# uci-cbcl/RP-Net

Hardware: AMD Instinct MI355X
Metric: support/query pairs/sec (fwd+bwd, 1-shot 256x256, T=5) (higher is better)
Workload: dtype f32

## Files before the change

rpnet_amd/csrc/bn.hip:

```cpp
#include <stdlib.h>

#include "common.h"
#include "lds_dma.h"
#include "split_bf16.h"

namespace rpnet {

struct BnGeom {
    int C4;
    int rows_it;
    int nblk;
    int rows_blk;
};

struct YSrc {
    const float* y;
};
__device__ __forceinline__ f32x4 load_y4(const YSrc s, const size_t off, const int) {
    return *reinterpret_cast<const f32x4*>(s.y + off);
}

static int bn_max_blocks(int C) { const int m = 131072 / C; return m < 256 ? 256 : (m > 1024 ? 1024 : m); }

static BnGeom bn_geom(long R, int C) {
// ... 176 lines not shown
                                                            const int C, const float sqrt_n, float* __restrict__ s_out) {
    RPNET_PASS_PRIORITY();
    __shared__ float red4[4];
    float m = 0.f;
    for (int c = threadIdx.x; c < C; c += 256) m = fmaxf(m, fabsf(gamma[c]) * sqrt_n + fabsf(beta[c]));
    m = block_max256(m, red4);
    if (threadIdx.x == 0) *s_out = pow2_scale(m);
}

template <int NP>
__global__ __launch_bounds__(256) void bn_relu_split_kernel(const YSrc ysrc, const float* __restrict__ scale,
                                                             const float* __restrict__ shift, float* __restrict__ z,
                                                             unsigned short* __restrict__ zs, size_t total8, int C8,
                                                             size_t group8, size_t plane_elems, const float* __restrict__ gamma,
                                                             const float* __restrict__ beta, const float sqrt_n,
                                                             float* __restrict__ s_out, const FastDiv fc, const FastDiv fg) {
    RPNET_PASS_PRIORITY();
    float inv_s = 1.f;
    if (NP <= 2) {
        __shared__ float red4[4];
        float m = 0.f;
        for (int c = threadIdx.x; c < C8 * 8; c += 256) m = fmaxf(m, fabsf(gamma[c]) * sqrt_n + fabsf(beta[c]));
        const float sc = pow2_scale(block_max256(m, red4));
        if (blockIdx.x == 0 && threadIdx.x == 0) *s_out = sc;
        inv_s = 1.f / sc;
    }
    for (size_t i = (size_t)blockIdx.x * 256 + threadIdx.x; i < total8; i += (size_t)gridDim.x * 256) {
        const int c8 = (int)fc.mod((unsigned)i);
        const int g = (int)fg.div((unsigned)i);
        const float* sc = scale + (size_t)(g * C8 + c8) * 8;
        const float* sh = shift + (size_t)(g * C8 + c8) * 8;
        float v[8];
#pragma unroll
        for (int hh = 0; hh < 2; ++hh) {
// ... 246 lines not shown
            for (int k = 0; k < 4; ++k) {
                const float m = fmaxf(fmaxf(a[k] * s4[k] + h4[k], b[k] * s4[k] + h4[k]), fmaxf(c[k] * s4[k] + h4[k], d[k] * s4[k] + h4[k]));
                o[k] = fmaxf(m, 0.f);
                v[hh * 4 + k] = o[k];
            }
            if (zp) reinterpret_cast<f32x4*>(zp)[i * 2 + hh] = o;
        }
        if (NP <= 2) {
#pragma unroll
            for (int k = 0; k < 8; ++k) v[k] *= inv_s;
        }
        u32x4 pl[NP];
        split8<NP>(v, pl);
#pragma unroll
        for (int p = 0; p < NP; ++p) *reinterpret_cast<u32x4*>(zs + p * plane_elems + i * 8) = pl[p];
    }
}

__device__ __forceinline__ int pool_argmax(const float a0, const float a1, const float a2, const float a3, float& best) {
    int q = 0; best = a0;
    if (a1 > best) { best = a1; q = 1; }
    if (a2 > best) { best = a2; q = 2; }
    if (a3 > best) { best = a3; q = 3; }
    return q;
}

template <int WIN>
__global__ __launch_bounds__(256) void bn_bwd_partial_pool(const float* __restrict__ dp, const YSrc ysrc,
                                                            const float* __restrict__ scale, const float* __restrict__ shift,
                                                            const float* __restrict__ mean, const float* __restrict__ invstd,
// ... 281 lines not shown
        else if (planes == 2) RPNET_BN_POOL(2);
        else RPNET_BN_POOL(1);
#undef RPNET_BN_POOL
        return check_launch("bn_relu_pool");
    }
    const size_t total4 = (size_t)N * HW * C / 4, group4 = total4 / groups;
    RPNET_REQUIRE(total4 < kIndex32, RPNET_ERR_SHAPE, "bn: %zu 16-byte elements do not fit the 32-bit index arithmetic of the passes", total4);
    if (z_split) {
        RPNET_REQUIRE(planes >= 1 && planes <= 3 && C % 8 == 0, RPNET_ERR_SHAPE, "bn_relu: split planes=%d C=%d", planes, C);
        const size_t total8 = total4 / 2, pe = (size_t)N * HW * C;
        RPNET_REQUIRE(planes == 3 || (gamma && beta && split_scale), RPNET_ERR_ARG,
                      "bn_relu: fp16 planes (1 or 2) need gamma, beta and the scale output");
        const float sqrt_n = sqrtf((float)((size_t)(N / groups) * HW)) * 1.0001f;
        if (planes == 3)
            hipLaunchKernelGGL(bn_relu_split_kernel<3>, dim3(elt_grid(total8)), dim3(256), 0, (hipStream_t)stream, ysrc, scale,
                               shift, z, (unsigned short*)z_split, total8, C / 8, group4 / 2, pe, gamma, beta, sqrt_n, split_scale, FastDiv(C / 8), FastDiv((unsigned)(group4 / 2)));
        else if (planes == 2)
            hipLaunchKernelGGL(bn_relu_split_kernel<2>, dim3(elt_grid(total8)), dim3(256), 0, (hipStream_t)stream, ysrc, scale,
                               shift, z, (unsigned short*)z_split, total8, C / 8, group4 / 2, pe, gamma, beta, sqrt_n, split_scale, FastDiv(C / 8), FastDiv((unsigned)(group4 / 2)));
        else
            hipLaunchKernelGGL(bn_relu_split_kernel<1>, dim3(elt_grid(total8)), dim3(256), 0, (hipStream_t)stream, ysrc, scale,
                               shift, z, (unsigned short*)z_split, total8, C / 8, group4 / 2, pe, gamma, beta, sqrt_n, split_scale, FastDiv(C / 8), FastDiv((unsigned)(group4 / 2)));
        return check_launch("bn_relu_split");
    }
    RPNET_REQUIRE(!split_scale || (gamma && beta), RPNET_ERR_ARG, "bn_relu: the tensor scale needs gamma and beta");
    hipLaunchKernelGGL(bn_relu_kernel, dim3(elt_grid(total4)), dim3(256), 0, (hipStream_t)stream, ysrc, scale, shift, z,
                       total4, C / 4, group4, gamma, beta, sqrtf((float)((size_t)(N / groups) * HW)) * 1.0001f, split_scale, FastDiv(C / 4),
                       FastDiv((unsigned)group4));
    return check_launch("bn_relu");
}

extern "C" int rpnet_bn_act_scale(const float* gamma, const float* beta, float* split_scale, int N, int HW, int C, int groups,
                                  rpnet_stream_t stream) {
    using namespace rpnet;
    RPNET_REQUIRE(gamma && beta && split_scale && groups >= 1 && C > 0, RPNET_ERR_ARG, "bn_act_scale: bad argument");
    hipLaunchKernelGGL(bn_act_scale_kernel, dim3(1), dim3(256), 0, (hipStream_t)stream, gamma, beta, C,
                       sqrtf((float)((size_t)(N / groups) * HW)) * 1.0001f, split_scale);
    return check_launch("bn_act_scale");
}

extern "C" int rpnet_bn_bwd(const float* dz, const float* y, const float* gamma, const float* scale, const float* shift,
                            const float* mean, const float* invstd, float* dy, void* dy_split, int planes, float* split_scale,
                            float* dgamma, float* dbeta, int N, int HW, int C, int groups, int accumulate,
                            const double* given_partial, const float* given_pmax, int given_rows, int pool_w, void* workspace,
                            size_t workspace_bytes, const float* y_dec, int y_dec_stride, rpnet_stream_t stream) {
    using namespace rpnet;
    (void)gamma;
    RPNET_REQUIRE(!y_dec && !y_dec_stride, RPNET_ERR_ARG, "bn_bwd: y_dec / y_dec_stride are reserved (must be NULL / 0)");
    const YSrc ysrc{y};
    RPNET_REQUIRE(dz && scale && shift && mean && invstd && dgamma && dbeta && workspace, RPNET_ERR_ARG, "bn_bwd: null pointer");
    RPNET_REQUIRE(y || (given_partial && !dy && !dy_split), RPNET_ERR_ARG, "bn_bwd: y is NULL but a pass that reads it was asked for");
    RPNET_REQUIRE(!dy_split || (planes >= 1 && planes <= 3 && C % 8 == 0), RPNET_ERR_SHAPE, "bn_bwd: split planes=%d C=%d",
                  planes, C);
// ... 140 lines not shown
```

rpnet_amd/functional.py:

```python
import collections
import contextlib
import ctypes as C
import os

import torch
from torch.autograd import Function
from torch.autograd.function import once_differentiable

from . import hip
from .hip import ConvDesc, call, ptr, query

BN_EPS = 1e-5
BN_MOMENTUM = 0.1

_ASYNC = {"on": False, "side": {}, "pending": set(), "queued": False, "fifo": [], "keep": []}

_MODES = {"f32": (0, False, 0), "bf16x3": (3, False, 0), "f16x2": (3, True, 2), "f16": (3, True, 1)}
_CORR_PRED_PLANES = True
_MATH = {}


def set_conv_math(mode):
    _MATH["mode"] = mode
    _MATH["planes"], _MATH["f16"], _MATH["f16_planes"] = _MODES[mode]
# ... 320 lines not shown
        if device is None or dv == device:
            for k in out:
                out[k] += pd[k]
    return out


def _empty(shape, like, dtype=torch.float32):
    return torch.empty(shape, device=like.device, dtype=dtype)


def _ws(nbytes, like):
    return torch.empty((max(int(nbytes), 16) + 7) // 8, device=like.device, dtype=torch.float64)


class Operand:
    __slots__ = ("x", "p16", "pbf", "scale", "planes_only", "deferred", "masked")

    def __init__(self, x, p16=None, pbf=None, scale=None, planes_only=False, deferred=None, masked=None):
        self.x, self.p16, self.pbf, self.scale = x, p16, pbf, scale
        self.deferred = deferred
        self.masked = masked
        self.planes_only = planes_only

    def values(self):
        if self.planes_only:
            raise RuntimeError("rpnet_amd: this operand exists as fp16 planes only (its producer was told that its single "
                               "consumer is a 3x3 convolution on fp16 planes); a consumer asked for the fp32 values")
        return self.x

    @property
    def shape(self):
        return self.x.shape

    def derive(self, x):
        return Operand(x, scale=self.scale)


_WGRAD_DEFER = 1
_EVAL_SPLITK = True
_POOL_FUSE = True
_CONV1_BN_FUSE = True
_CONV1_RECOMP = True
_UP4 = True
_MASK_SKIP = os.environ.get("RPNET_MASK_SKIP", "1") == "1"


_SKIP_STATS = None


def _set_skip(d, mask, mode, halo, N, H, W, on=None):
    if (_MASK_SKIP if on is None else on) and mask is not None and mode in (1, 2):
        if _SKIP_STATS is not None:
            d._skip_ws = torch.full((max(N * H * W // 128, 16),), 255, device=mask.device, dtype=torch.uint8)
            _SKIP_STATS.append(d._skip_ws)
        else:
            d._skip_ws = torch.empty(max(N * H * W // 128, 16), device=mask.device, dtype=torch.uint8)
        d.skip_mask, d.skip_mode, d.skip_halo, d.skip_ws = ptr(mask), mode, halo, ptr(d._skip_ws)
        ARITH[("zero_tile_skip", "armed")] += 1

# ... 50 lines not shown
        return None
    masked = in_scale is not None and in_mode
    fp = _MATH["f16_planes"]

    def ready(op):
        return op.p16 is not None and op.p16.shape[1:] == op.x.shape and op.p16.shape[0] == fp

    if op1 is None and not masked and ready(op0):
        return op0.p16, None, s0, None
    pre = op0.masked
    if (op1 is None and masked and pre is not None and pre[0] is in_scale and pre[1] == in_mode and pre[2].shape[0] == fp
            and pre[2].dtype == torch.float16):
        return pre[2], None, s0, None
    if two_scales and op1 is not None and not masked and ready(op0) and ready(op1):
        return op0.p16, op1.p16, s0, s1
    xs0, s = split_f16(op0.values(), s0, s1, in_scale if masked else None, in_mode if masked else 0)
    xs1 = split_f16(op1.values(), s0, s1, want_scale=False)[0] if op1 is not None else None
    if op1 is None and not masked:
        op0.p16 = xs0
    return xs0, xs1, s, None


class PackedWeight:

    def __init__(self, weight, split=None, pool=None):
        cout, cin, kh, kw = weight.shape
        self._pool = pool
        self.taps = kh * kw
        if split is None:
            self.off0, self.split, self.off1, self.cin_pad = 0, cin, cin, cin
# ... 201 lines not shown

def _dgrad_desc(pw, dys, sdy, dy, g0, g1, N, H, W, out_scale=None, out_mode=0, up4=False, skippable=False, skip_on=None):
    if dys is None:
        return _desc(dy, None, pw.wd, None, None, 0, g0, g1, N, H, W, pw.taps, 0, out_scale=out_scale, out_mode=out_mode)
    np_ = dys.shape[0]
    pk = pw.up4_packs(np_) if up4 else pw.split_packs(np_)
    dd = _desc(dys, None, pk[1], None, None, 0, g0, g1, N, H, W, pw.taps, 1 if up4 else 0, out_scale=out_scale, out_mode=out_mode)
    dd.split_planes = np_
    if np_ <= 2:
        dd.acc_scale_col, dd.acc_scale_x = ptr(pk[3]), ptr(sdy)
        if skippable:
            _set_skip(dd, out_scale, out_mode, 0, N, H, W, skip_on)
    return dd


_Req = collections.namedtuple("_Req", "z_unused pool pool_req defer_act eval_grad")


class _Produced:
    __slots__ = ("p16", "pbf", "scale", "planes_only", "deferred", "pooled")

    def __init__(self):
        self.p16 = self.pbf = self.scale = self.deferred = None
        self.planes_only = self.pooled = False


_State = collections.namedtuple("_State", "shape groups bias beta bn_eval pool pw upsample in_mode xs sx sx1 up4 async_on skip_on")


def _save_state(ctx, saved=None, shape=None, groups=1, bias=None, beta=None, bn_eval=False, pool=False, pw=None, upsample=0, in_mode=0, plan=None):
    if saved is None:
        ctx.st = None
        return
    ctx.save_for_backward(*saved)
    split = plan is not None and plan.planes
    ctx.st = _State(shape, groups, bias, beta, bn_eval, pool, pw, upsample, in_mode, plan.xs if split else None,
                    plan.sx if split else None, plan.sx1 if split else None, plan is not None and plan.kind == "up4", _ASYNC["on"], _MASK_SKIP)

# ... 46 lines not shown
             BN_EPS, ptr(stats[0]), ptr(stats[1]), ptr(stats[2]), ptr(stats[3]), ptr(ws), wsb)
    _order_done(gamma.data_ptr())
    return stats


def _bn_output(y, stats, shape, groups, gamma, beta, out_split, req, res, pool_ok, conv1=None):
    N, H, W, cout = shape
    planes_out = out_split in (True, "corr")
    want16 = _want16(cout, out_split)
    np_out = 0
    if planes_out and cout % 32 == 0 and _MATH["planes"]:
        np_out = _MATH["f16_planes"] if want16 else _MATH["planes"]
    pool = res.pooled = bool(pool_ok and np_out > 0 and out_split is True and H % 2 == 0 and W % 2 == 0)
    Hz, Wz = (H // 2, W // 2) if pool else (H, W)
    dev = gamma.device
    zs = torch.empty((np_out, N, Hz, Wz, cout), device=dev, dtype=torch.float16 if np_out <= 2 else torch.bfloat16) if np_out else None
    sz = torch.empty(1, device=dev, dtype=torch.float32) if want16 else None
    if req.z_unused and want16 and np_out and (pool or not req.pool_req):
        z = torch.empty(1, device=dev, dtype=torch.float32).expand(N, Hz, Wz, cout)
        res.planes_only = True
    else:
        z = torch.empty((N, Hz, Wz, cout), device=dev, dtype=torch.float32)
    if req.defer_act and not (pool or np_out or want16 or res.planes_only) and conv1 is None and groups == 1:
        res.deferred = (y, stats[0], stats[1])
    elif conv1 is not None:
        if not (res.planes_only and np_out):
            raise RuntimeError("rpnet_amd: the first layer was run without its pre-BatchNorm tensor but its output is not planes-only")
        call("rpnet_conv1_bn_relu", ptr(conv1[0]), ptr(conv1[1]), ptr(conv1[2]), ptr(stats[0]), ptr(stats[1]), None, ptr(zs), np_out,
             ptr(gamma), ptr(beta), ptr(sz), N, H, W, cout, groups)
        ARITH[("bn_relu", "first layer made again from the image")] += 1
# ... 319 lines not shown
        if fuse:
            call("rpnet_conv1_wgrad_bn", ptr(x0), ptr(dz), ptr(y), ptr(stats), coef, ptr(dw), N, H, W, cout, groups, ptr(ws2), wb, *again)
        else:
            call("rpnet_conv1_wgrad", ptr(x0), ptr(dy), ptr(dw), N, H, W, cout, ptr(ws2), wb)
        dw = _accumulate_direct(weight, dw, st.async_on)
        dx0 = None
        if ctx.needs_input_grad[0]:
            dx0 = _empty(x0.shape, dz)
            call("rpnet_conv1_dgrad_bn", ptr(dz), ptr(y), ptr(stats), coef, ptr(weight), again[1], ptr(x0) if y is None else None,
                 ptr(dx0), N, H, W, cout, groups)
        db = _bias_grad(bias, gamma, stats, dbeta, st.bn_eval, st.async_on)
        return dx0, dw, db, dgamma, dbeta, None, None, None, None


def conv_bn_relu_op(x0, conv, bn, cache, training, x1=None, in_scale=None, in_mode=0, groups=1, upsample=False, split=None,
                    out_split=True, z_unused=False, pool=False, defer_act=False):
    op0, op1 = as_operand(x0), as_operand(x1)
    w = conv.weight
    x1t = None if op1 is None else op1.x
    eval_grad = not training and torch.is_grad_enabled() and any(
        t is not None and t.requires_grad for t in (op0.x, x1t, in_scale, w, conv.bias, bn.weight, bn.bias))
    req = _Req(bool(z_unused) and training and w.shape[0] % 64 == 0, bool(pool) and training and _POOL_FUSE, bool(pool),
               bool(defer_act) and training and not out_split, eval_grad)
    res = _Produced()
    bnbuf = (bn.running_mean, bn.running_var, bn.num_batches_tracked if training else None)
    if w.shape[1] == 1 and w.shape[2] == 3:
        if x1t is not None or in_scale is not None or upsample:
            raise RuntimeError("rpnet_amd: the first-layer convolution takes one plain source (no second source, mask or up-sampling)")
        z = Conv1BnRelu.apply(op0.x, w, conv.bias, bn.weight, bn.bias, bnbuf, (training, groups, out_split), req, res)
    else:
        pw = cache.get(w, split)
        z = ConvBnRelu.apply(op0.x, x1t, in_scale, w, conv.bias, bn.weight, bn.bias, bnbuf, pw,
                             (training, groups, 1 if upsample else 0, in_mode, out_split), (op0, op1), req, res)
    out = Operand(z, res.p16, res.pbf, res.scale, res.planes_only, res.deferred)
    if pool and not res.pooled:
        out = maxpool2(out)
    return out


def conv_bn_relu(x0, conv, bn, cache, training, **kw):
    return conv_bn_relu_op(x0, conv, bn, cache, training, **kw).x


class ConvRelu(Function):

    @staticmethod
    def forward(ctx, x, weight, bias, pw, relu, dilation):
        hip.require_gpu(x, weight)
        N, H, W, _ = x.shape
# ... 122 lines not shown
                dst.zero_()
                continue
            for i in range(0, len(live), 15):
                chunk = ([dst] if i else []) + live[i:i + 15]
                if len(chunk) == 1:
                    dst.copy_(chunk[0])
                else:
                    arr = (C.c_void_p * len(chunk))(*[t.data_ptr() for t in chunk])
                    call("rpnet_sum_n", arr, len(chunk), ptr(dst), dst.numel())
        return out, None, None, None


class PoolSkip(Function):

    @staticmethod
    def forward(ctx, z):
        N, H, W, Cc = z.shape
        out = _empty((N, H // 2, W // 2, Cc), z)
        call("rpnet_maxpool2_fwd", ptr(z), ptr(out), N, H, W, Cc)
        ctx.save_for_backward(z)
        return z.view_as(z), out

    @staticmethod
    @once_differentiable
    def backward(ctx, dskip, dpool):
        if dpool is None:
            return dskip
        (z,) = ctx.saved_tensors
        N, H, W, Cc = z.shape
        dz = torch.empty_like(z)
        call("rpnet_maxpool2_bwd", ptr(z), ptr(dpool.contiguous()), None if dskip is None else ptr(dskip.contiguous()), ptr(dz),
             N, H, W, Cc)
        return dz


def pool_skip(op):
    op = as_operand(op)
    z, pooled = PoolSkip.apply(op.values())
    return Operand(z, p16=op.p16, pbf=op.pbf, scale=op.scale), op.derive(pooled)


class MaxPool2(Function):

    @staticmethod
    def forward(ctx, z):
        N, H, W, Cc = z.shape
        out = _empty((N, H // 2, W // 2, Cc), z)
        call("rpnet_maxpool2_fwd", ptr(z), ptr(out), N, H, W, Cc)
        ctx.save_for_backward(z)
        return out

    @staticmethod
    @once_differentiable
# ... 389 lines not shown
```

rpnet_amd/hip.py:

```python
import ctypes as C
import os

import torch

_LIB_PATH = os.environ.get("RPNET_LIB_PATH") or os.path.join(os.path.dirname(os.path.abspath(__file__)), "librpnet_hip.so")
_lib = None

vp, ci, cf, cs, cd = C.c_void_p, C.c_int, C.c_float, C.c_size_t, C.c_double


class ConvDesc(C.Structure):
    _fields_ = [("x0", vp), ("x1", vp), ("C0", ci), ("C1", ci), ("w", vp), ("bias", vp), ("in_scale", vp),
                ("in_scale_mode", ci), ("y0", vp), ("y1", vp), ("Co0", ci), ("Co1", ci), ("ep_scale", vp),
                ("ep_shift", vp), ("ep_relu", ci), ("out_scale", vp), ("out_scale_mode", ci), ("accumulate", ci),
                ("N", ci), ("H", ci), ("W", ci), ("taps", ci), ("upsample", ci), ("groups", ci), ("dilation", ci), ("stats_partial", vp), ("split_planes", ci), ("y_split", vp), ("split_out_planes", ci),
                ("acc_scale_col", vp), ("acc_scale_x", vp), ("acc_scale_dy", vp), ("bnb_y", vp), ("bnb_stats", vp), ("bnb_partial", vp), ("bnb_pmax", vp), ("bnb_groups", ci),
                ("acc_scale_x1", vp), ("out_absmax", vp), ("tune", ci), ("y_split_scale", vp), ("splitk_ws", vp), ("splitk_ws_bytes", cs),
                ("skip_mask", vp), ("skip_mode", ci), ("skip_halo", ci), ("skip_ws", vp), ("tile_skip", vp),
                ("y_enc", vp), ("y_enc_stride", ci)]


PACK_MAX = 24


# ... 134 lines not shown
    "rpnet_surface_workspace_bytes": (cs, [ci, ci, ci]),
    "rpnet_surface_tally": (ci, [vp, ci, vp, ci, ci, ci, ci, ci, vp, C.c_int64, vp, C.c_int64, C.c_int64, vp, cs, vp]),
}
SURFACE_ABI_SYMBOLS = tuple(_SURFACE_SIGS)
SURFACE_ABI_VERSION = 1

_CC_SIGS = {
    "rpnet_cc_abi_version": (ci, []),
    "rpnet_cc_workspace_bytes": (cs, [ci, ci, ci]),
    "rpnet_cc_label": (ci, [vp, ci, ci, ci, ci, ci, ci, vp, vp, C.c_int64, C.c_int64, vp, cs, vp]),
    "rpnet_cc_keep_largest": (ci, [vp, ci, vp, ci, ci, ci, ci, ci, vp, ci, vp, C.c_int64, vp, C.c_int64, C.c_int64, vp, cs, vp]),
}
CC_ABI_SYMBOLS = tuple(_CC_SIGS)
CC_ABI_VERSION = 1


def lib_path():
    return _LIB_PATH


def load():
    global _lib
    if _lib is None:
        if not os.path.exists(_LIB_PATH):
            raise RuntimeError(f"{_LIB_PATH} not found: build it with `make -C rpnet_amd/csrc` "
                               "(or __graft_entry__.build()); rpnet_amd has no CPU fallback")
        lib = C.CDLL(_LIB_PATH)
        lib.rpnet_version.restype = ci
        if lib.rpnet_version() != ABI_VERSION:
            raise RuntimeError(f"{_LIB_PATH} has ABI version {lib.rpnet_version()}, this binding was written for {ABI_VERSION} "
                               "(include/rpnet_abi.h RPNET_ABI_VERSION): rebuild it with `make -C rpnet_amd/csrc`")
        for name, (res, args) in (list(_SIGS.items()) + list(_EVAL_SIGS.items()) + list(_OPTIM_SIGS.items()) + list(_GUARD_SIGS.items())
                                  + list(_SURFACE_SIGS.items()) + list(_CC_SIGS.items())):
            fn = getattr(lib, name, None)
            if fn is None:
                raise RuntimeError(f"{_LIB_PATH} does not export {name}: rebuild it with `make -C rpnet_amd/csrc`")
            fn.restype, fn.argtypes = res, args
        if lib.rpnet_eval_abi_version() != EVAL_ABI_VERSION:
            raise RuntimeError(f"{_LIB_PATH} has evaluation-item ABI version {lib.rpnet_eval_abi_version()}, this binding was written for "
                               f"{EVAL_ABI_VERSION} (include/rpnet_eval_abi.h): rebuild it with `make -C rpnet_amd/csrc`")
        if lib.rpnet_optim_abi_version() != OPTIM_ABI_VERSION:
            raise RuntimeError(f"{_LIB_PATH} has optimizer ABI version {lib.rpnet_optim_abi_version()}, this binding was written for "
                               f"{OPTIM_ABI_VERSION} (include/rpnet_optim_abi.h): rebuild it with `make -C rpnet_amd/csrc`")
        if lib.rpnet_guard_abi_version() != GUARD_ABI_VERSION:
            raise RuntimeError(f"{_LIB_PATH} has gradient-guard ABI version {lib.rpnet_guard_abi_version()}, this binding was written for "
                               f"{GUARD_ABI_VERSION} (include/rpnet_guard_abi.h): rebuild it with `make -C rpnet_amd/csrc`")
        if lib.rpnet_surface_abi_version() != SURFACE_ABI_VERSION:
            raise RuntimeError(f"{_LIB_PATH} has surface-distance ABI version {lib.rpnet_surface_abi_version()}, this binding was written "
                               f"for {SURFACE_ABI_VERSION} (include/rpnet_surface_abi.h): rebuild it with `make -C rpnet_amd/csrc`")
        if lib.rpnet_cc_abi_version() != CC_ABI_VERSION:
            raise RuntimeError(f"{_LIB_PATH} has connected-component ABI version {lib.rpnet_cc_abi_version()}, this binding was written "
                               f"for {CC_ABI_VERSION} (include/rpnet_cc_abi.h): rebuild it with `make -C rpnet_amd/csrc`")
        _lib = lib
    return _lib


def ptr(t):
    return None if t is None else t.data_ptr()


try:
    _raw_stream, _cur_device = torch._C._cuda_getCurrentRawStream, torch._C._cuda_getDevice
except AttributeError:
    _raw_stream = None


def stream():
# ... 22 lines not shown
```

rpnet_amd/modules.py:

```python
import itertools
import os

import torch
import torch.nn as nn

from . import functional as RF
from .schedule import Schedule

_FANIN = 2
_PREPACK = True
_ZSKIP = True
_F16_MIN_PIXELS = int(os.environ.get("RPNET_F16_MIN_PIXELS", "262144"))
_F16_MIN_PIXELS_EVAL = int(os.environ.get("RPNET_F16_MIN_PIXELS_EVAL", "524288"))
_CRE_STREAMS = True
_CRE_STREAMS_MAX_PIXELS = 16384
_CRE_STREAMS_TRAIN = os.environ.get("RPNET_CRE_STREAMS_TRAIN", "1") == "1"
_ENC_STREAMS = int(os.environ.get("RPNET_ENC_STREAMS", "1"))
_NET_SERIAL = itertools.count(1)


def _to_nhwc(x):
    return x.permute(0, 2, 3, 1).contiguous()


# ... 27 lines not shown
    return training, groups


class conv_block(nn.Module):

    def __init__(self, ch_in, ch_out, normalization_type, kernel=3, padding=1):
        super().__init__()
        assert kernel == 3 and padding == 1
        self.ch_in, self.ch_out = ch_in, ch_out
        self.conv = nn.Sequential(
            nn.Conv2d(ch_in, ch_out, kernel_size=kernel, stride=1, padding=padding, bias=True),
            _norm(normalization_type, ch_out), nn.ReLU(inplace=True),
            nn.Conv2d(ch_out, ch_out, kernel_size=kernel, stride=1, padding=padding, bias=True),
            _norm(normalization_type, ch_out), nn.ReLU(inplace=True))

    def forward_nhwc(self, x0, cache, x1=None, groups=1, out_split=True, split=None, pool=False):
        t, groups = _norm_mode(self.conv[1], self.training, groups, x0)
        x = RF.conv_bn_relu_op(x0, self.conv[0], self.conv[1], cache, t, x1=x1, groups=groups, z_unused=_ZSKIP, split=split)
        if pool:
            return RF.conv_bn_relu_op(x, self.conv[3], self.conv[4], cache, t, groups=groups, out_split=True, z_unused=_ZSKIP,
                                      pool=True)
        return RF.conv_bn_relu_op(x, self.conv[3], self.conv[4], cache, t, groups=groups, out_split=out_split)

    def forward(self, x):
        return _to_nchw(self.forward_nhwc(_to_nhwc(x), RF.WeightCache()).x)


class up_conv(nn.Module):

    def __init__(self, ch_in, ch_out, normalization_type, kernel=3, padding=1):
        super().__init__()
        assert kernel == 3 and padding == 1
        self.ch_in, self.ch_out = ch_in, ch_out
        self.up = nn.Sequential(
            nn.Upsample(scale_factor=2),
            nn.Conv2d(ch_in, ch_out, kernel_size=kernel, stride=1, padding=padding, bias=True),
            _norm(normalization_type, ch_out), nn.ReLU(inplace=True))

    def forward_nhwc(self, x, cache, groups=1, out_split=True):
        t, groups = _norm_mode(self.up[2], self.training, groups, x)
        return RF.conv_bn_relu_op(x, self.up[1], self.up[2], cache, t, groups=groups, upsample=True, out_split=out_split)

    def forward(self, x):
        return _to_nchw(self.forward_nhwc(_to_nhwc(x), RF.WeightCache()).x)


class Unet_2D(nn.Module):

    def __init__(self, cfg, img_ch=5, output_ch=6, t=2, pretrained=True, resnet_type="resnet18"):
        super().__init__()
        self.cfg = cfg
        self.img_ch, self.t, self.pretrained, self.resnet_type = img_ch, t, pretrained, resnet_type
        self.final_activation = cfg["final_activation"]
        self.output_ch = output_ch

    def set_mode(self, mode):
# ... 27 lines not shown
    def _mask_source(self, mask, scale):
        m = RF.mask_avgpool(mask, scale) if scale > 1 else mask
        src = torch.zeros(*m.shape, 64, device=m.device, dtype=torch.float32)
        src[..., 0] = m
        return RF.Operand(src, scale=torch.full((1,), 2.0 ** -15, device=m.device, dtype=torch.float32))

    def forward_nhwc(self, x, cache, groups=1, mask=None):
        if x.shape[1] % 16 or x.shape[2] % 16:
            raise ValueError(f"U_Net needs H, W multiples of 16, got {tuple(x.shape[1:3])}")
        mfm = self.mask_feature_map
        if mfm and mask is None:
            raise ValueError(f"mask_feature_map={mfm!r} needs the mask")
        pool = RF.maxpool2
        sk = "scale" if RF.f16_mode() else True
        f1, f2 = self.training and mfm != "x2", self.training and mfm != "x3"
        if mfm == "x":
            xin = torch.zeros(*x.shape[:3], 64, device=x.device, dtype=torch.float32)
            xin[..., 0], xin[..., 1] = x[..., 0], mask.float()
            p1 = self.Conv1.forward_nhwc(xin, cache, groups=groups, out_split=sk, split=(2, 64, 64), pool=f1)
        else:
            p1 = self.Conv1.forward_nhwc(x, cache, groups=groups, out_split=sk, pool=f1)
        if not f1:
            p1 = pool(p1)
        if mfm == "x2":
            p2 = self.Conv2.forward_nhwc(p1, cache, x1=self._mask_source(mask.float(), 2), groups=groups, out_split=sk,
                                         split=(64, 64, 128), pool=f2)
        else:
            p2 = self.Conv2.forward_nhwc(p1, cache, groups=groups, out_split=sk, pool=f2)
        if not f2:
            p2 = pool(p2)
        if mfm == "x3":
            x3 = self.Conv3.forward_nhwc(p2, cache, x1=self._mask_source(mask.float(), 4), groups=groups, out_split=sk,
                                         split=(128, 128, 192))
        else:
            x3 = self.Conv3.forward_nhwc(p2, cache, groups=groups, out_split=sk)
        sch = getattr(self, "schedule", None)
        fan = (_FANIN if sch is None else sch.get("fanin", _FANIN)) >= 2 and torch.is_grad_enabled() and x3.x.requires_grad
        x3, p3 = RF.pool_skip(x3) if fan else (x3, pool(x3))
        x4 = self.Conv4.forward_nhwc(p3, cache, groups=groups, out_split=sk)
        x4, p4 = RF.pool_skip(x4) if fan else (x4, pool(x4))
        x5 = self.Conv5.forward_nhwc(p4, cache, groups=groups)
        d5 = self.Up5.forward_nhwc(x5, cache, groups=groups, out_split=sk)
        d5 = self.Up_conv5.forward_nhwc(x4, cache, x1=d5, groups=groups)
        d4 = self.Up4.forward_nhwc(d5, cache, groups=groups, out_split=sk)
        return self.Up_conv4.forward_nhwc(x3, cache, x1=d4, groups=groups, out_split=sk)

    def forward(self, x, mask=None, do_last_conv=True):
        n, c, h, w = x.shape
        assert c == 1
        m = None if mask is None else mask.reshape(n, h, w)
        return {"d4": _to_nchw(self.forward_nhwc(x.reshape(n, h, w, 1), RF.WeightCache(), mask=m).x)}


class Encoder(nn.Module):

    def __init__(self, in_channels=3, pretrained_path=None):
        super().__init__()
        self.pretrained_path = pretrained_path
        self.features = nn.Sequential(
# ... 386 lines not shown
```

rpnet_amd/schedule.py:

```python
import dataclasses
from typing import Optional


@dataclasses.dataclass
class Schedule:
    conv_math: Optional[str] = None
    async_wgrad: Optional[bool] = None
    mask_skip: Optional[bool] = None
    cre_streams_train: Optional[bool] = None
    cre_streams_eval: Optional[bool] = None
    enc_streams: Optional[int] = None
    fanin: Optional[int] = None
    f16_min_pixels: Optional[int] = None
    f16_min_pixels_eval: Optional[int] = None

    def get(self, name, default):
        v = getattr(self, name)
        return default if v is None else v

    def overrides(self):
        return {f.name: getattr(self, f.name) for f in dataclasses.fields(self) if getattr(self, f.name) is not None}
```

Before: 493.8.

## Fuse BN-ReLU with skip max-pool and share joint fp16 plane scales

Adds a fused BN+ReLU+2x2 pool kernel that writes the full-resolution activation, the pooled fp16 planes and optionally the full-resolution planes in one pass. Conv3 and Conv4 outputs then skip the separate maxpool and plane-split passes in the fan-in path. A joint scale kernel computes one shared power-of-two scale for each skip tensor and its matching decoder upsample output, so the concatenated operands of the Up_conv layers can reuse planes without rescaling. The cost is extra code paths, more kernel variants, and a slightly coarser shared scale for the fp16 planes.

```diff
diff --git a/include/rpnet_planes_abi.h b/include/rpnet_planes_abi.h
--- /dev/null
+++ b/include/rpnet_planes_abi.h
@@ -0,0 +1,26 @@
+#ifndef RPNET_PLANES_ABI_H
+#define RPNET_PLANES_ABI_H
+
+#include <stddef.h>
+
+#include "rpnet_abi.h"
+
+#ifdef __cplusplus
+extern "C" {
+#endif
+
+#define RPNET_PLANES_ABI_VERSION 1
+int rpnet_planes_abi_version(void);
+
+int rpnet_bn_joint_scale(const float* gamma_a, const float* beta_a, int N_a, int HW_a, int C_a, int groups_a, const float* gamma_b,
+                         const float* beta_b, int N_b, int HW_b, int C_b, int groups_b, float* scales3, rpnet_stream_t stream);
+int rpnet_bn_relu_at_scale(const float* y, const float* scale, const float* shift, float* z, void* z_split, int planes,
+                           const float* plane_scale, int N, int HW, int C, int groups, rpnet_stream_t stream);
+int rpnet_bn_relu_skip_pool(const float* y, const float* scale, const float* shift, float* z, void* pool_split, void* full_split,
+                            int planes, const float* pool_scale, const float* full_scale, int N, int HW, int C, int groups, int pool_w,
+                            rpnet_stream_t stream);
+
+#ifdef __cplusplus
+}
+#endif
+#endif
diff --git a/rpnet_amd/csrc/bn.hip b/rpnet_amd/csrc/bn.hip
--- a/rpnet_amd/csrc/bn.hip
+++ b/rpnet_amd/csrc/bn.hip
@@ -2,6 +2,7 @@
 
 #include "common.h"
 #include "lds_dma.h"
+#include "rpnet_planes_abi.h"
 #include "split_bf16.h"
 
 namespace rpnet {
@@ -214,10 +215,13 @@
                                                              unsigned short* __restrict__ zs, size_t total8, int C8,
                                                              size_t group8, size_t plane_elems, const float* __restrict__ gamma,
                                                              const float* __restrict__ beta, const float sqrt_n,
-                                                             float* __restrict__ s_out, const FastDiv fc, const FastDiv fg) {
+                                                             float* __restrict__ s_out, const FastDiv fc, const FastDiv fg,
+                                                             const float* __restrict__ s_ext) {
     RPNET_PASS_PRIORITY();
     float inv_s = 1.f;
-    if (NP <= 2) {
+    if (NP <= 2 && s_ext) {
+        inv_s = 1.f / *s_ext;
+    } else if (NP <= 2) {
         __shared__ float red4[4];
         float m = 0.f;
         for (int c = threadIdx.x; c < C8 * 8; c += 256) m = fmaxf(m, fabsf(gamma[c]) * sqrt_n + fabsf(beta[c]));
@@ -494,6 +498,88 @@
         split8<NP>(v, pl);
 #pragma unroll
         for (int p = 0; p < NP; ++p) *reinterpret_cast<u32x4*>(zs + p * plane_elems + i * 8) = pl[p];
+    }
+}
+
+template <int NP, bool FULL, bool DRAIN>
+__global__ __launch_bounds__(256) void bn_relu_skip_pool_split_kernel(const YSrc ysrc, const float* __restrict__ scale,
+                                                                       const float* __restrict__ shift, float* __restrict__ z,
+                                                                       unsigned short* __restrict__ zps, unsigned short* __restrict__ zfs,
+                                                                       size_t total8, int C8, PoolGeom pg, size_t pool_plane_elems,
+                                                                       size_t full_plane_elems, const float* __restrict__ s_pool,
+                                                                       const float* __restrict__ s_full) {
+    static_assert(NP <= 2, "fp16 planes only: a scale handed in by pointer");
+    const float inv_p = 1.f / *s_pool;
+    const float inv_f = FULL ? 1.f / *s_full : 1.f;
+    const size_t rowC = (size_t)pg.W * C8 * 8;
+    for (size_t i = (size_t)blockIdx.x * 256 + threadIdx.x; i < total8; i += (size_t)gridDim.x * 256) {
+        unsigned pp, py, pn;
+        const int c8 = (int)pg.fC8.divmod((unsigned)i, pp);
+        const int ox = (int)pg.fWo.divmod(pp, py);
+        const int oy = (int)pg.fHo.divmod(py, pn);
+        const int n = (int)pn;
+        const int g = (int)pg.fIpg.div(pn);
+        const float* sc = scale + (size_t)(g * C8 + c8) * 8;
+        const float* sh = shift + (size_t)(g * C8 + c8) * 8;
+        const size_t src = (size_t)n * pg.img_elems + ((size_t)(2 * oy) * pg.W + 2 * ox) * C8 * 8 + c8 * 8;
+        const size_t offs[4] = {src, src + (size_t)C8 * 8, src + rowC, src + rowC + (size_t)C8 * 8};
+        float vp[8], vf[4][8];
+#pragma unroll
+        for (int hh = 0; hh < 2; ++hh) {
+            const int cc = c8 * 8 + hh * 4;
+            f32x4 a = load_y4(ysrc, offs[0] + hh * 4, cc);
+            f32x4 b = load_y4(ysrc, offs[1] + hh * 4, cc);
+            f32x4 c = load_y4(ysrc, offs[2] + hh * 4, cc);
+            f32x4 d = load_y4(ysrc, offs[3] + hh * 4, cc);
+            f32x4 s4 = reinterpret_cast<const f32x4*>(sc)[hh], h4 = reinterpret_cast<const f32x4*>(sh)[hh];
+            if constexpr (DRAIN) asm volatile("s_waitcnt vmcnt(0)" : "+v"(a), "+v"(b), "+v"(c), "+v"(d), "+v"(s4), "+v"(h4) : : "memory");
+            f32x4 zq[4];
+#pragma unroll
+            for (int k = 0; k < 4; ++k) {
+                zq[0][k] = fmaxf(a[k] * s4[k] + h4[k], 0.f);
+                zq[1][k] = fmaxf(b[k] * s4[k] + h4[k], 0.f);
+                zq[2][k] = fmaxf(c[k] * s4[k] + h4[k], 0.f);
+                zq[3][k] = fmaxf(d[k] * s4[k] + h4[k], 0.f);
+                vp[hh * 4 + k] = fmaxf(fmaxf(zq[0][k], zq[1][k]), fmaxf(zq[2][k], zq[3][k])) * inv_p;
+            }
+#pragma unroll
+            for (int q = 0; q < 4; ++q) {
+                *reinterpret_cast<f32x4*>(z + offs[q] + hh * 4) = zq[q];
+                if constexpr (FULL) {
+#pragma unroll
+                    for (int k = 0; k < 4; ++k) vf[q][hh * 4 + k] = zq[q][k] * inv_f;
+                }
+            }
+        }
+        u32x4 pl[NP];
+        split8<NP>(vp, pl);
+#pragma unroll
+        for (int p = 0; p < NP; ++p) *reinterpret_cast<u32x4*>(zps + p * pool_plane_elems + i * 8) = pl[p];
+        if constexpr (FULL) {
+#pragma unroll
+            for (int q = 0; q < 4; ++q) {
+                split8<NP>(vf[q], pl);
+#pragma unroll
+                for (int p = 0; p < NP; ++p) *reinterpret_cast<u32x4*>(zfs + p * full_plane_elems + offs[q]) = pl[p];
+            }
+        }
+    }
+}
+
+__global__ __launch_bounds__(256) void bn_joint_scale_kernel(const float* __restrict__ gamma_a, const float* __restrict__ beta_a,
+                                                              const int Ca, const float sqrt_na, const float* __restrict__ gamma_b,
+                                                              const float* __restrict__ beta_b, const int Cb, const float sqrt_nb,
+                                                              float* __restrict__ s) {
+    RPNET_PASS_PRIORITY();
+    __shared__ float red4[4];
+    float ma = 0.f, mb = 0.f;
+    for (int c = threadIdx.x; c < Ca; c += 256) ma = fmaxf(ma, fabsf(gamma_a[c]) * sqrt_na + fabsf(beta_a[c]));
+    for (int c = threadIdx.x; c < Cb; c += 256) mb = fmaxf(mb, fabsf(gamma_b[c]) * sqrt_nb + fabsf(beta_b[c]));
+    ma = block_max256(ma, red4);
+    mb = block_max256(mb, red4);
+    if (threadIdx.x == 0) {
+        const float sa = pow2_scale(ma), sb = pow2_scale(mb);
+        s[0] = sa; s[1] = sb; s[2] = fmaxf(sa, sb);
     }
 }
 
@@ -805,13 +891,13 @@
         const float sqrt_n = sqrtf((float)((size_t)(N / groups) * HW)) * 1.0001f;
         if (planes == 3)
             hipLaunchKernelGGL(bn_relu_split_kernel<3>, dim3(elt_grid(total8)), dim3(256), 0, (hipStream_t)stream, ysrc, scale,
-                               shift, z, (unsigned short*)z_split, total8, C / 8, group4 / 2, pe, gamma, beta, sqrt_n, split_scale, FastDiv(C / 8), FastDiv((unsigned)(group4 / 2)));
+                               shift, z, (unsigned short*)z_split, total8, C / 8, group4 / 2, pe, gamma, beta, sqrt_n, split_scale, FastDiv(C / 8), FastDiv((unsigned)(group4 / 2)), (const float*)nullptr);
         else if (planes == 2)
             hipLaunchKernelGGL(bn_relu_split_kernel<2>, dim3(elt_grid(total8)), dim3(256), 0, (hipStream_t)stream, ysrc, scale,
-                               shift, z, (unsigned short*)z_split, total8, C / 8, group4 / 2, pe, gamma, beta, sqrt_n, split_scale, FastDiv(C / 8), FastDiv((unsigned)(group4 / 2)));
+                               shift, z, (unsigned short*)z_split, total8, C / 8, group4 / 2, pe, gamma, beta, sqrt_n, split_scale, FastDiv(C / 8), FastDiv((unsigned)(group4 / 2)), (const float*)nullptr);
         else
             hipLaunchKernelGGL(bn_relu_split_kernel<1>, dim3(elt_grid(total8)), dim3(256), 0, (hipStream_t)stream, ysrc, scale,
-                               shift, z, (unsigned short*)z_split, total8, C / 8, group4 / 2, pe, gamma, beta, sqrt_n, split_scale, FastDiv(C / 8), FastDiv((unsigned)(group4 / 2)));
+                               shift, z, (unsigned short*)z_split, total8, C / 8, group4 / 2, pe, gamma, beta, sqrt_n, split_scale, FastDiv(C / 8), FastDiv((unsigned)(group4 / 2)), (const float*)nullptr);
         return check_launch("bn_relu_split");
     }
     RPNET_REQUIRE(!split_scale || (gamma && beta), RPNET_ERR_ARG, "bn_relu: the tensor scale needs gamma and beta");
@@ -828,6 +914,76 @@
     hipLaunchKernelGGL(bn_act_scale_kernel, dim3(1), dim3(256), 0, (hipStream_t)stream, gamma, beta, C,
                        sqrtf((float)((size_t)(N / groups) * HW)) * 1.0001f, split_scale);
     return check_launch("bn_act_scale");
+}
+
+extern "C" int rpnet_planes_abi_version(void) { return RPNET_PLANES_ABI_VERSION; }
+
+static float bn_bound_sqrt_n(int N, int HW, int groups) { return sqrtf((float)((size_t)(N / groups) * HW)) * 1.0001f; }
+
+extern "C" int rpnet_bn_joint_scale(const float* gamma_a, const float* beta_a, int N_a, int HW_a, int C_a, int groups_a,
+                                    const float* gamma_b, const float* beta_b, int N_b, int HW_b, int C_b, int groups_b,
+                                    float* scales3, rpnet_stream_t stream) {
+    using namespace rpnet;
+    RPNET_REQUIRE(gamma_a && beta_a && gamma_b && beta_b && scales3, RPNET_ERR_ARG, "bn_joint_scale: null pointer");
+    RPNET_REQUIRE(C_a > 0 && C_b > 0 && HW_a > 0 && HW_b > 0 && groups_a >= 1 && groups_b >= 1 && N_a >= groups_a && N_b >= groups_b &&
+                  N_a % groups_a == 0 && N_b % groups_b == 0, RPNET_ERR_SHAPE,
+                  "bn_joint_scale: N=%d/%d HW=%d/%d C=%d/%d groups=%d/%d", N_a, N_b, HW_a, HW_b, C_a, C_b, groups_a, groups_b);
+    hipLaunchKernelGGL(bn_joint_scale_kernel, dim3(1), dim3(256), 0, (hipStream_t)stream, gamma_a, beta_a, C_a,
+                       bn_bound_sqrt_n(N_a, HW_a, groups_a), gamma_b, beta_b, C_b, bn_bound_sqrt_n(N_b, HW_b, groups_b), scales3);
+    return check_launch("bn_joint_scale");
+}
+
+extern "C" int rpnet_bn_relu_at_scale(const float* y, const float* scale, const float* shift, float* z, void* z_split, int planes,
+                                      const float* plane_scale, int N, int HW, int C, int groups, rpnet_stream_t stream) {
+    using namespace rpnet;
+    RPNET_REQUIRE(y && scale && shift && z_split && plane_scale, RPNET_ERR_ARG, "bn_relu_at_scale: null pointer");
+    RPNET_REQUIRE((planes == 1 || planes == 2) && C % 8 == 0 && C > 0 && HW > 0, RPNET_ERR_SHAPE,
+                  "bn_relu_at_scale: planes=%d (1 or 2: fp16) C=%d (a multiple of 8) HW=%d", planes, C, HW);
+    if (int rc = bn_check("bn_relu_at_scale", N, HW, C, groups)) return rc;
+    const YSrc ysrc{y};
+    const size_t total8 = (size_t)N * HW * C / 8, group8 = total8 / groups, pe = (size_t)N * HW * C;
+    RPNET_REQUIRE(total8 > 0 && total8 * 2 < kIndex32, RPNET_ERR_SHAPE,
+                  "bn_relu_at_scale: %zu 16-byte elements do not fit the 32-bit index arithmetic of the passes", total8 * 2);
+    if (planes == 2)
+        hipLaunchKernelGGL(bn_relu_split_kernel<2>, dim3(elt_grid(total8)), dim3(256), 0, (hipStream_t)stream, ysrc, scale, shift, z,
+                           (unsigned short*)z_split, total8, C / 8, group8, pe, (const float*)nullptr, (const float*)nullptr, 0.f,
+                           (float*)nullptr, FastDiv(C / 8), FastDiv((unsigned)group8), plane_scale);
+    else
+        hipLaunchKernelGGL(bn_relu_split_kernel<1>, dim3(elt_grid(total8)), dim3(256), 0, (hipStream_t)stream, ysrc, scale, shift, z,
+                           (unsigned short*)z_split, total8, C / 8, group8, pe, (const float*)nullptr, (const float*)nullptr, 0.f,
+                           (float*)nullptr, FastDiv(C / 8), FastDiv((unsigned)group8), plane_scale);
+    return check_launch("bn_relu_at_scale");
+}
+
+extern "C" int rpnet_bn_relu_skip_pool(const float* y, const float* scale, const float* shift, float* z, void* pool_split,
+                                       void* full_split, int planes, const float* pool_scale, const float* full_scale, int N, int HW,
+                                       int C, int groups, int pool_w, rpnet_stream_t stream) {
+    using namespace rpnet;
+    RPNET_REQUIRE(y && scale && shift && z && pool_split && pool_scale, RPNET_ERR_ARG, "bn_relu_skip_pool: null pointer");
+    RPNET_REQUIRE(!full_split == !full_scale, RPNET_ERR_ARG, "bn_relu_skip_pool: the full-resolution planes and their scale go together");
+    RPNET_REQUIRE((planes == 1 || planes == 2) && C % 8 == 0 && C > 0, RPNET_ERR_SHAPE,
+                  "bn_relu_skip_pool: planes=%d (1 or 2: fp16) C=%d (a multiple of 8)", planes, C);
+    if (int rc = bn_check("bn_relu_skip_pool", N, HW, C, groups)) return rc;
+    RPNET_REQUIRE(pool_w > 0 && HW > 0 && HW % pool_w == 0 && pool_w % 2 == 0 && (HW / pool_w) % 2 == 0, RPNET_ERR_SHAPE,
+                  "bn_relu_skip_pool: pooled image %d x %d", pool_w > 0 ? HW / pool_w : 0, pool_w);
+    const YSrc ysrc{y};
+    const PoolGeom pg = make_pool_geom(HW, pool_w, N, groups, C);
+    const size_t total8 = (size_t)N * (HW / 4) * C / 8, pe = (size_t)N * (HW / 4) * C, fe = (size_t)N * HW * C;
+    RPNET_REQUIRE(total8 > 0 && total8 < kIndex32, RPNET_ERR_SHAPE,
+                  "bn_relu_skip_pool: %zu elements do not fit the 32-bit index arithmetic of the passes", total8);
+    const size_t alone_f = pool_alone_bytes();
+    static const bool drain_f = [] { const char* e = getenv("RPNET_BN_POOL_DRAIN"); return !(e && e[0] == '0'); }();
+#define RPNET_BN_SKIP_POOL(NP_, FULL_)                                                                                             \
+    do { if (drain_f) hipLaunchKernelGGL((bn_relu_skip_pool_split_kernel<NP_, FULL_, true>), dim3(elt_grid(total8)), dim3(256), alone_f, \
+                       (hipStream_t)stream, ysrc, scale, shift, z, (unsigned short*)pool_split, (unsigned short*)full_split, total8, \
+                       C / 8, pg, pe, fe, pool_scale, full_scale);                                                                 \
+    else hipLaunchKernelGGL((bn_relu_skip_pool_split_kernel<NP_, FULL_, false>), dim3(elt_grid(total8)), dim3(256), alone_f,       \
+                       (hipStream_t)stream, ysrc, scale, shift, z, (unsigned short*)pool_split, (unsigned short*)full_split, total8, \
+                       C / 8, pg, pe, fe, pool_scale, full_scale); } while (0)
+    if (planes == 2) { if (full_split) RPNET_BN_SKIP_POOL(2, true); else RPNET_BN_SKIP_POOL(2, false); }
+    else { if (full_split) RPNET_BN_SKIP_POOL(1, true); else RPNET_BN_SKIP_POOL(1, false); }
+#undef RPNET_BN_SKIP_POOL
+    return check_launch("bn_relu_skip_pool");
 }
 
 extern "C" int rpnet_bn_bwd(const float* dz, const float* y, const float* gamma, const float* scale, const float* shift,
diff --git a/rpnet_amd/functional.py b/rpnet_amd/functional.py
--- a/rpnet_amd/functional.py
+++ b/rpnet_amd/functional.py
@@ -358,10 +358,11 @@
 
 
 class Operand:
-    __slots__ = ("x", "p16", "pbf", "scale", "planes_only", "deferred", "masked")
-
-    def __init__(self, x, p16=None, pbf=None, scale=None, planes_only=False, deferred=None, masked=None):
+    __slots__ = ("x", "p16", "pbf", "scale", "planes_only", "deferred", "masked", "joint", "pool_p16")
+
+    def __init__(self, x, p16=None, pbf=None, scale=None, planes_only=False, deferred=None, masked=None, joint=None, pool_p16=None):
         self.x, self.p16, self.pbf, self.scale = x, p16, pbf, scale
+        self.joint, self.pool_p16 = joint, pool_p16
         self.deferred = deferred
         self.masked = masked
         self.planes_only = planes_only
@@ -387,6 +388,19 @@
 _CONV1_RECOMP = True
 _UP4 = True
 _MASK_SKIP = os.environ.get("RPNET_MASK_SKIP", "1") == "1"
+_PLANE_FUSE = os.environ.get("RPNET_PLANE_FUSE", "1") == "1"
+
+
+class JointScale:
+    __slots__ = ("t", "a", "b", "joint")
+
+    def __init__(self, bn_a, bn_b, N, HW, groups):
+        ga, gb = bn_a.weight, bn_b.weight
+        hip.require_gpu(ga, gb)
+        self.t = torch.empty(3, device=ga.device, dtype=torch.float32)
+        call("rpnet_bn_joint_scale", ptr(ga), ptr(bn_a.bias), N, HW, ga.shape[0], groups, ptr(gb), ptr(bn_b.bias), N, HW, gb.shape[0],
+             groups, ptr(self.t))
+        self.a, self.b, self.joint = self.t[0:1], self.t[1:2], self.t[2:3]
 
 
 _SKIP_STATS = None
@@ -467,6 +481,10 @@
         return pre[2], None, s0, None
     if two_scales and op1 is not None and not masked and ready(op0) and ready(op1):
         return op0.p16, op1.p16, s0, s1
+    jn = op0.joint
+    if (op1 is not None and not masked and jn is not None and jn[1] is s1 and ready(op1) and jn[0].shape[0] == fp
+            and jn[0].shape[1:] == op0.x.shape):
+        return jn[0], op1.p16, s1, None
     xs0, s = split_f16(op0.values(), s0, s1, in_scale if masked else None, in_mode if masked else 0)
     xs1 = split_f16(op1.values(), s0, s1, want_scale=False)[0] if op1 is not None else None
     if op1 is None and not masked:
@@ -698,14 +716,14 @@
     return dd
 
 
-_Req = collections.namedtuple("_Req", "z_unused pool pool_req defer_act eval_grad")
+_Req = collections.namedtuple("_Req", "z_unused pool pool_req defer_act eval_grad skip_pool plane_scale", defaults=(None, None))
 
 
 class _Produced:
-    __slots__ = ("p16", "pbf", "scale", "planes_only", "deferred", "pooled")
+    __slots__ = ("p16", "pbf", "scale", "planes_only", "deferred", "pooled", "joint", "pool_p16")
 
     def __init__(self):
-        self.p16 = self.pbf = self.scale = self.deferred = None
+        self.p16 = self.pbf = self.scale = self.deferred = self.joint = self.pool_p16 = None
         self.planes_only = self.pooled = False
 
 
@@ -782,6 +800,25 @@
     pool = res.pooled = bool(pool_ok and np_out > 0 and out_split is True and H % 2 == 0 and W % 2 == 0)
     Hz, Wz = (H // 2, W // 2) if pool else (H, W)
     dev = gamma.device
+    fp = _MATH["f16_planes"]
+    fuse16 = want16 and out_split == "scale" and conv1 is None and fp in (1, 2) and cout % 64 == 0
+    if fuse16 and req.skip_pool is not None and H % 2 == 0 and W % 2 == 0:
+        js = req.skip_pool
+        res.pool_p16 = torch.empty((fp, N, H // 2, W // 2, cout), device=dev, dtype=torch.float16)
+        full = torch.empty((fp, N, H, W, cout), device=dev, dtype=torch.float16)
+        z = torch.empty((N, H, W, cout), device=dev, dtype=torch.float32)
+        call("rpnet_bn_relu_skip_pool", ptr(y), ptr(stats[0]), ptr(stats[1]), ptr(z), ptr(res.pool_p16), ptr(full), fp, ptr(js.a),
+             ptr(js.joint), N, H * W, cout, groups, W)
+        ARITH[("bn_planes", "with the pooled and the skip planes")] += 1
+        res.joint, res.scale = (full, js.joint), js.a
+        return z
+    if fuse16 and req.plane_scale is not None:
+        res.p16 = torch.empty((fp, N, H, W, cout), device=dev, dtype=torch.float16)
+        call("rpnet_bn_relu_at_scale", ptr(y), ptr(stats[0]), ptr(stats[1]), None, ptr(res.p16), fp, ptr(req.plane_scale), N, H * W, cout,
+             groups)
+        ARITH[("bn_planes", "planes on the consumer's scale")] += 1
+        res.scale, res.planes_only = req.plane_scale, True
+        return torch.empty(1, device=dev, dtype=torch.float32).expand(N, H, W, cout)
     zs = torch.empty((np_out, N, Hz, Wz, cout), device=dev, dtype=torch.float16 if np_out <= 2 else torch.bfloat16) if np_out else None
     sz = torch.empty(1, device=dev, dtype=torch.float32) if want16 else None
     if req.z_unused and want16 and np_out and (pool or not req.pool_req):
@@ -1131,14 +1168,15 @@
 
 
 def conv_bn_relu_op(x0, conv, bn, cache, training, x1=None, in_scale=None, in_mode=0, groups=1, upsample=False, split=None,
-                    out_split=True, z_unused=False, pool=False, defer_act=False):
+                    out_split=True, z_unused=False, pool=False, defer_act=False, skip_pool=None, plane_scale=None):
     op0, op1 = as_operand(x0), as_operand(x1)
     w = conv.weight
     x1t = None if op1 is None else op1.x
     eval_grad = not training and torch.is_grad_enabled() and any(
         t is not None and t.requires_grad for t in (op0.x, x1t, in_scale, w, conv.bias, bn.weight, bn.bias))
     req = _Req(bool(z_unused) and training and w.shape[0] % 64 == 0, bool(pool) and training and _POOL_FUSE, bool(pool),
-               bool(defer_act) and training and not out_split, eval_grad)
+               bool(defer_act) and training and not out_split, eval_grad, skip_pool if training else None,
+               plane_scale if training else None)
     res = _Produced()
     bnbuf = (bn.running_mean, bn.running_var, bn.num_batches_tracked if training else None)
     if w.shape[1] == 1 and w.shape[2] == 3:
@@ -1149,7 +1187,7 @@
         pw = cache.get(w, split)
         z = ConvBnRelu.apply(op0.x, x1t, in_scale, w, conv.bias, bn.weight, bn.bias, bnbuf, pw,
                              (training, groups, 1 if upsample else 0, in_mode, out_split), (op0, op1), req, res)
-    out = Operand(z, res.p16, res.pbf, res.scale, res.planes_only, res.deferred)
+    out = Operand(z, res.p16, res.pbf, res.scale, res.planes_only, res.deferred, joint=res.joint, pool_p16=res.pool_p16)
     if pool and not res.pooled:
         out = maxpool2(out)
     return out
@@ -1302,10 +1340,13 @@
 class PoolSkip(Function):
 
     @staticmethod
-    def forward(ctx, z):
+    def forward(ctx, z, pooled_exists=False):
         N, H, W, Cc = z.shape
-        out = _empty((N, H // 2, W // 2, Cc), z)
-        call("rpnet_maxpool2_fwd", ptr(z), ptr(out), N, H, W, Cc)
+        if pooled_exists:
+            out = torch.empty(1, device=z.device, dtype=torch.float32).expand(N, H // 2, W // 2, Cc)
+        else:
+            out = _empty((N, H // 2, W // 2, Cc), z)
+            call("rpnet_maxpool2_fwd", ptr(z), ptr(out), N, H, W, Cc)
         ctx.save_for_backward(z)
         return z.view_as(z), out
 
@@ -1313,18 +1354,22 @@
     @once_differentiable
     def backward(ctx, dskip, dpool):
         if dpool is None:
-            return dskip
+            return dskip, None
         (z,) = ctx.saved_tensors
         N, H, W, Cc = z.shape
         dz = torch.empty_like(z)
         call("rpnet_maxpool2_bwd", ptr(z), ptr(dpool.contiguous()), None if dskip is None else ptr(dskip.contiguous()), ptr(dz),
              N, H, W, Cc)
-        return dz
+        return dz, None
 
 
 def pool_skip(op):
     op = as_operand(op)
-    z, pooled = PoolSkip.apply(op.values())
+    if op.pool_p16 is not None:
+        z, pooled = PoolSkip.apply(op.values(), True)
+        return (Operand(z, p16=op.p16, pbf=op.pbf, scale=op.scale, joint=op.joint),
+                Operand(pooled, p16=op.pool_p16, scale=op.scale, planes_only=True))
+    z, pooled = PoolSkip.apply(op.values(), False)
     return Operand(z, p16=op.p16, pbf=op.pbf, scale=op.scale), op.derive(pooled)
 
 
diff --git a/rpnet_amd/hip.py b/rpnet_amd/hip.py
--- a/rpnet_amd/hip.py
+++ b/rpnet_amd/hip.py
@@ -172,6 +172,15 @@
 CC_ABI_SYMBOLS = tuple(_CC_SIGS)
 CC_ABI_VERSION = 1
 
+_PLANES_SIGS = {
+    "rpnet_planes_abi_version": (ci, []),
+    "rpnet_bn_joint_scale": (ci, [vp, vp, ci, ci, ci, ci, vp, vp, ci, ci, ci, ci, vp, vp]),
+    "rpnet_bn_relu_at_scale": (ci, [vp, vp, vp, vp, vp, ci, vp, ci, ci, ci, ci, vp]),
+    "rpnet_bn_relu_skip_pool": (ci, [vp, vp, vp, vp, vp, vp, ci, vp, vp, ci, ci, ci, ci, ci, vp]),
+}
+PLANES_ABI_SYMBOLS = tuple(_PLANES_SIGS)
+PLANES_ABI_VERSION = 1
+
 
 def lib_path():
     return _LIB_PATH
@@ -189,7 +198,7 @@
             raise RuntimeError(f"{_LIB_PATH} has ABI version {lib.rpnet_version()}, this binding was written for {ABI_VERSION} "
                                "(include/rpnet_abi.h RPNET_ABI_VERSION): rebuild it with `make -C rpnet_amd/csrc`")
         for name, (res, args) in (list(_SIGS.items()) + list(_EVAL_SIGS.items()) + list(_OPTIM_SIGS.items()) + list(_GUARD_SIGS.items())
-                                  + list(_SURFACE_SIGS.items()) + list(_CC_SIGS.items())):
+                                  + list(_SURFACE_SIGS.items()) + list(_CC_SIGS.items()) + list(_PLANES_SIGS.items())):
             fn = getattr(lib, name, None)
             if fn is None:
                 raise RuntimeError(f"{_LIB_PATH} does not export {name}: rebuild it with `make -C rpnet_amd/csrc`")
@@ -209,6 +218,9 @@
         if lib.rpnet_cc_abi_version() != CC_ABI_VERSION:
             raise RuntimeError(f"{_LIB_PATH} has connected-component ABI version {lib.rpnet_cc_abi_version()}, this binding was written "
                                f"for {CC_ABI_VERSION} (include/rpnet_cc_abi.h): rebuild it with `make -C rpnet_amd/csrc`")
+        if lib.rpnet_planes_abi_version() != PLANES_ABI_VERSION:
+            raise RuntimeError(f"{_LIB_PATH} has operand-plane ABI version {lib.rpnet_planes_abi_version()}, this binding was written "
+                               f"for {PLANES_ABI_VERSION} (include/rpnet_planes_abi.h): rebuild it with `make -C rpnet_amd/csrc`")
         _lib = lib
     return _lib
 
diff --git a/rpnet_amd/modules.py b/rpnet_amd/modules.py
--- a/rpnet_amd/modules.py
+++ b/rpnet_amd/modules.py
@@ -65,13 +65,13 @@
             nn.Conv2d(ch_out, ch_out, kernel_size=kernel, stride=1, padding=padding, bias=True),
             _norm(normalization_type, ch_out), nn.ReLU(inplace=True))
 
-    def forward_nhwc(self, x0, cache, x1=None, groups=1, out_split=True, split=None, pool=False):
+    def forward_nhwc(self, x0, cache, x1=None, groups=1, out_split=True, split=None, pool=False, skip_pool=None):
         t, groups = _norm_mode(self.conv[1], self.training, groups, x0)
         x = RF.conv_bn_relu_op(x0, self.conv[0], self.conv[1], cache, t, x1=x1, groups=groups, z_unused=_ZSKIP, split=split)
         if pool:
             return RF.conv_bn_relu_op(x, self.conv[3], self.conv[4], cache, t, groups=groups, out_split=True, z_unused=_ZSKIP,
                                       pool=True)
-        return RF.conv_bn_relu_op(x, self.conv[3], self.conv[4], cache, t, groups=groups, out_split=out_split)
+        return RF.conv_bn_relu_op(x, self.conv[3], self.conv[4], cache, t, groups=groups, out_split=out_split, skip_pool=skip_pool)
 
     def forward(self, x):
         return _to_nchw(self.forward_nhwc(_to_nhwc(x), RF.WeightCache()).x)
@@ -88,9 +88,10 @@
             nn.Conv2d(ch_in, ch_out, kernel_size=kernel, stride=1, padding=padding, bias=True),
             _norm(normalization_type, ch_out), nn.ReLU(inplace=True))
 
-    def forward_nhwc(self, x, cache, groups=1, out_split=True):
+    def forward_nhwc(self, x, cache, groups=1, out_split=True, plane_scale=None):
         t, groups = _norm_mode(self.up[2], self.training, groups, x)
-        return RF.conv_bn_relu_op(x, self.up[1], self.up[2], cache, t, groups=groups, upsample=True, out_split=out_split)
+        return RF.conv_bn_relu_op(x, self.up[1], self.up[2], cache, t, groups=groups, upsample=True, out_split=out_split,
+                                  plane_scale=plane_scale)
 
     def forward(self, x):
         return _to_nchw(self.forward_nhwc(_to_nhwc(x), RF.WeightCache()).x)
@@ -148,6 +149,15 @@
         pool = RF.maxpool2
         sk = "scale" if RF.f16_mode() else True
         f1, f2 = self.training and mfm != "x2", self.training and mfm != "x3"
+        sch = getattr(self, "schedule", None)
+        fan_on = (_FANIN if sch is None else sch.get("fanin", _FANIN)) >= 2 and torch.is_grad_enabled()
+        j3 = j4 = None
+        plain = not mfm and not any(getattr(m, "instance", False) for m in (self.Conv3.conv[4], self.Conv4.conv[4], self.Up5.up[2], self.Up4.up[2]))
+        fuse = RF._PLANE_FUSE if sch is None else sch.get("plane_fuse", RF._PLANE_FUSE)
+        if fuse and fan_on and self.training and plain and x.is_cuda and RF.f16_mode() and RF.pack_planes() in (1, 2):
+            n, hq, wq = x.shape[0], x.shape[1] // 4, x.shape[2] // 4
+            j3 = RF.JointScale(self.Conv3.conv[4], self.Up4.up[2], n, hq * wq, groups)
+            j4 = RF.JointScale(self.Conv4.conv[4], self.Up5.up[2], n, (hq // 2) * (wq // 2), groups)
         if mfm == "x":
             xin = torch.zeros(*x.shape[:3], 64, device=x.device, dtype=torch.float32)
             xin[..., 0], xin[..., 1] = x[..., 0], mask.float()
@@ -167,16 +177,15 @@
             x3 = self.Conv3.forward_nhwc(p2, cache, x1=self._mask_source(mask.float(), 4), groups=groups, out_split=sk,
                                          split=(128, 128, 192))
         else:
-            x3 = self.Conv3.forward_nhwc(p2, cache, groups=groups, out_split=sk)
-        sch = getattr(self, "schedule", None)
-        fan = (_FANIN if sch is None else sch.get("fanin", _FANIN)) >= 2 and torch.is_grad_enabled() and x3.x.requires_grad
+            x3 = self.Conv3.forward_nhwc(p2, cache, groups=groups, out_split=sk, skip_pool=j3)
+        fan = fan_on and x3.x.requires_grad
         x3, p3 = RF.pool_skip(x3) if fan else (x3, pool(x3))
-        x4 = self.Conv4.forward_nhwc(p3, cache, groups=groups, out_split=sk)
+        x4 = self.Conv4.forward_nhwc(p3, cache, groups=groups, out_split=sk, skip_pool=j4)
         x4, p4 = RF.pool_skip(x4) if fan else (x4, pool(x4))
         x5 = self.Conv5.forward_nhwc(p4, cache, groups=groups)
-        d5 = self.Up5.forward_nhwc(x5, cache, groups=groups, out_split=sk)
+        d5 = self.Up5.forward_nhwc(x5, cache, groups=groups, out_split=sk, plane_scale=x4.joint[1] if x4.joint else None)
         d5 = self.Up_conv5.forward_nhwc(x4, cache, x1=d5, groups=groups)
-        d4 = self.Up4.forward_nhwc(d5, cache, groups=groups, out_split=sk)
+        d4 = self.Up4.forward_nhwc(d5, cache, groups=groups, out_split=sk, plane_scale=x3.joint[1] if x3.joint else None)
         return self.Up_conv4.forward_nhwc(x3, cache, x1=d4, groups=groups, out_split=sk)
 
     def forward(self, x, mask=None, do_last_conv=True):
diff --git a/rpnet_amd/schedule.py b/rpnet_amd/schedule.py
--- a/rpnet_amd/schedule.py
+++ b/rpnet_amd/schedule.py
@@ -13,6 +13,7 @@
     fanin: Optional[int] = None
     f16_min_pixels: Optional[int] = None
     f16_min_pixels_eval: Optional[int] = None
+    plane_fuse: Optional[bool] = None
 
     def get(self, name, default):
         v = getattr(self, name)
```

Result: no change. 496.1, median of 6 (+0.5%).
